# NumericalEarth/Breeze.jl

Measured on AMD Instinct MI355X. Metric: grid-cells advanced/sec (tendency+Poisson step), 512^3 anelastic, higher is better.
Workload: dtype f64

## Files before the change

breeze.jl_amd/csrc/bz_tendency5_kernels.h:

```cpp
#pragma once
#include "bz_internal.h"
#include "bz_weno.h"
#include "bz_tendency3_kernels.h"

#ifndef BZ_KO
#define BZ_KO 0
#endif
#ifndef BZ6_ROTATE_DUTY
#define BZ6_ROTATE_DUTY 0
#endif
#ifndef BZ6_UNROLL2
#define BZ6_UNROLL2 0
#endif
#ifndef BZ6_LDS_BARRIER
#define BZ6_LDS_BARRIER 0
#endif
__device__ __forceinline__ void bz6_barrier()
{
#if BZ6_LDS_BARRIER
    __builtin_amdgcn_fence(__ATOMIC_RELEASE, "workgroup", "local");
    __builtin_amdgcn_s_barrier();
    __builtin_amdgcn_fence(__ATOMIC_ACQUIRE, "workgroup", "local");
#else
    __syncthreads();
#endif
}
typedef long long ix_t;
typedef unsigned ix32_t;

struct LevRow5 {
    double rho, rrho;
    double rho_f, rrho_f;
    double Ax, Ay, Vinv_c;
    double pi;
    double Vinv_f, T_r;
    double pad[6];
};
struct Lev5 {
    const LevRow5 *p;
#ifdef __HIPCC__
    __device__ __forceinline__ double at(int k, int f) const { return ((ColPtr::cptr)(const double *)p)[(long long)k * 16 + f]; }
    __device__ __forceinline__ double rho(int k) const { return at(k, 0); }
    __device__ __forceinline__ double rrho(int k) const { return at(k, 1); }
    __device__ __forceinline__ double rho_f(int k) const { return at(k, 2); }
    __device__ __forceinline__ double rrho_f(int k) const { return at(k, 3); }
    __device__ __forceinline__ double Ax(int k) const { return at(k, 4); }
    __device__ __forceinline__ double Ay(int k) const { return at(k, 5); }
    __device__ __forceinline__ double Vinv_c(int k) const { return at(k, 6); }
    __device__ __forceinline__ double pi(int k) const { return at(k, 7); }
    __device__ __forceinline__ double Vinv_f(int k) const { return at(k, 8); }
// ... 197 lines not shown
    {
        const double rh = g.rho[kbeg], rr = g.rrho[kbeg];
        bool z0 = (b[3] == 0.0);
#pragma unroll
        for (int q = 0; q < HPT; ++q)
            if (hok[q]) {
                T[0][0][hr[q]][hc[q]] = bz_cdiv(pa[hn[q]], rh, rr);
                if constexpr (Q) {
                    const double hbv = bz_cdiv(pb[hn[q]], rh, rr);
                    T[0][1][hr[q]][hc[q]] = hbv;
                    z0 = z0 && (hbv == 0.0);
                }
            }
        if (ZS && !__all(z0) && tx == 0) ZF[0] = 0;
    }
    __syncthreads();

    double ea = 0.0, eb = 0.0;
    int buf = 0;
    double ru_n = ru[n], rv_n = rv[n], rw_n = rw[n + sz];
    double rvtop_n = (tyu == 0 || (Q && tyu == TY / 2)) ? rv[ntop0] : 0.0;
    double ta_nx = 0.0, tb_nx = 0.0;
    if constexpr (BZ5_TOPS_AHEAD) { ta_nx = pa[n + 3 * sz]; if constexpr (Q) tb_nx = pb[n + 3 * sz]; }
    for (int k = kbeg; k < kend; ++k, n += sz) {
        double ha[HPT], hb[HPT];
        const unsigned lev = (unsigned)(k + 1 - kbeg) * sz;
        double ta_raw, tb_raw = 0.0;
        if constexpr (BZ5_TOPS_AHEAD) {
            ta_raw = ta_nx; tb_raw = tb_nx;
            const unsigned up = (k + 4 <= g.Nz + g.Hz - 1) ? 4 * sz : 3 * sz;
            ta_nx = pa[n + up];
            if constexpr (Q) tb_nx = pb[n + up];
        } else { ta_raw = pa[n + 3 * sz]; if constexpr (Q) tb_raw = pb[n + 3 * sz]; }
        const int lv3 = (ZS || (Q && BZ5_RAW_LDS)) ? (k - kbeg) % 3 : 0;
        bool zxy = false;
        if constexpr (ZS) {
            if (t == 0) ZF[(lv3 + 2) % 3] = 1;
            zxy = __builtin_amdgcn_readfirstlane(ZF[lv3]) != 0;
        }
#pragma unroll
        for (int q = 0; q < HPT; ++q) {
            if (BZ_KO & 2) { ha[q] = ta_raw; hb[q] = tb_raw; }
            else { ha[q] = hok[q] ? pa[hn[q] + lev] : 0.0; hb[q] = (Q && hok[q]) ? pb[hn[q] + lev] : 0.0; }
        }
        const double u0a = (BZ_KO & 16) ? ta_raw : (E.mode == 2) ? E.u0[n] : 0.0, u0b = (BZ_KO & 16) ? tb_raw : (Q && E.mode == 2) ? E.u0b[n] : 0.0;
        const double ru_t = ru_n, rv_t = rv_n, rw_t = rw_n, rvtop = rvtop_n;
        const int turn = (k - kbeg) & (TY - 1);
        const bool duty_a = tyu == turn, duty_b = Q && tyu == ((turn + TY / 2) & (TY - 1));
        if (BZ_KO & 32) { ru_n = ta_raw * 1e-3; rv_n = tb_raw; rw_n = ta_raw * 1e-4; } else {
        ru_n = ru[n + sz]; rv_n = rv[n + sz]; rw_n = rw[n + 2 * sz]; }
        {
            const int turn_n = (turn + 1) & (TY - 1);
            const bool duty_n = tyu == turn_n || (Q && tyu == ((turn_n + TY / 2) & (TY - 1)));
            rvtop_n = duty_n ? rv[ntop0 + lev] : 0.0;
        }
        const double rho = LV.rho(k), rrho = LV.rrho(k), Ax_k = LV.Ax(k), Ay_k = LV.Ay(k), Vi_k = LV.Vinv_c(k);
        const double rho1 = LV.rho(k + 1), rrho1 = LV.rrho(k + 1), rhof1 = LV.rho_f(k + 1), rrhof1 = LV.rrho_f(k + 1);
        const double rho3 = LV.rho(k + 3), rrho3 = LV.rrho(k + 3);
        if (((k - kbeg) & (BZ5_EB - 1)) == 0) {
            const int kk = min(k + (tx & (BZ5_EB - 1)), kend - 1);
            const long long ne = g.idx(ie, jc, kk);
            const double rhk = g.rho[kk], rrk = g.rrho[kk];
            const double ue = bz_cdiv(ru[ne], rhk, rrk);
            const bool le_ = ue > 0.0;
            const double cf = g.Ax[kk] * ue;
            ea = rhk * (cf * bz_up5(bz_cdiv(pa[ne - 3], rhk, rrk), bz_cdiv(pa[ne - 2], rhk, rrk), bz_cdiv(pa[ne - 1], rhk, rrk),
                                    bz_cdiv(pa[ne], rhk, rrk), bz_cdiv(pa[ne + 1], rhk, rrk), bz_cdiv(pa[ne + 2], rhk, rrk), le_));
            if constexpr (Q)
            eb = rhk * (cf * bz_up5(bz_cdiv(pb[ne - 3], rhk, rrk), bz_cdiv(pb[ne - 2], rhk, rrk), bz_cdiv(pb[ne - 1], rhk, rrk),
                                    bz_cdiv(pb[ne], rhk, rrk), bz_cdiv(pb[ne + 1], rhk, rrk), bz_cdiv(pb[ne + 2], rhk, rrk), le_));
        }
        const int src = (k - kbeg) & (BZ5_EB - 1);
        const double ut = bz_cdiv(ru_t, rho, rrho), vt = bz_cdiv(rv_t, rho, rrho);
        const double wt = bz_cdiv(rw_t, rhof1, rrhof1);
        const double cfx = Ax_k * ut, cfy = Ay_k * vt, cfz = g.Az * wt, rf = rhof1;
        const bool lx = ut > 0.0, ly = vt > 0.0, lz = wt > 0.0;
        const int Bz = bz_buffer_face(k + 1, g.Nz);
        double cfy2 = 0.0;
        bool ly2 = false;
        if (duty_a || duty_b) {
            const double vtop = bz_cdiv(rvtop, rho, rrho);
            ly2 = vtop > 0.0;
            cfy2 = Ay_k * vtop;
        }
        const int c = tx + 3;
        double fxa, fya, fza_hi, fxb, fyb, fzb_hi;
        const double ta = bz_cdiv(ta_raw, rho3, rrho3);
        {
            const double(*Tk)[TC] = T[buf][0];
            const double *rr_ = Tk[ty + 3] + tx;
            fxa = rho * (cfx * bz_up5(rr_[0], rr_[1], rr_[2], a[3], rr_[4], rr_[5], lx));
            fya = rho * (cfy * bz_up5y<WY>(Tk[ty][c], Tk[ty + 1][c], Tk[ty + 2][c], a[3], Tk[ty + 4][c], Tk[ty + 5][c], ly, Byj));
            FY[buf][0][ty][tx] = fya;
            if (duty_a)
                FY[buf][0][TY][tx] = rho * (cfy2 * bz_up5y<WY>(Tk[TY][c], Tk[TY + 1][c], Tk[TY + 2][c], Tk[TY + 3][c], Tk[TY + 4][c], Tk[TY + 5][c], ly2, Byt));
            fza_hi = rf * (cfz * bz_upB(a[1], a[2], a[3], a[4], a[5], ta, lz, Bz));
        }
        double tb = 0.0;
        fxb = 0.0; fyb = 0.0; fzb_hi = 0.0;
        if constexpr (Q) {
// ... 55 lines not shown
            const double ga = -(Vi * ((na - fxa) + dya + (fza_hi - fza)));
            double gb = 0.0;
            if constexpr (Q) {
                double nb = __shfl_down(fxb, 1);
                const double xb = __shfl(eb, src);
                if (tx == le) nb = xb;
                const double dyb = FY[buf][1][ty + 1][tx] - fyb;
                gb = -(Vi * ((nb - fxb) + dyb + (fzb_hi - fzb)));
            }
            if (store) {
                const double rth = bz_rk_apply_pre(E.mode, E.dt, E.alpha, E.oma, u0a, E.u0_out, ga, pa_n, n);
                F.oa[n] = rth;
                if constexpr (Q) {
                    const double rq = bz_rk_apply_pre(E.mode, E.dt, E.alpha, E.oma, u0b, E.u0b_out, gb, pb_n, n);
                    F.ob[n] = rq;
                }
            }
        }
        fza = fza_hi; fzb = fzb_hi;
#pragma unroll
        for (int s = 0; s < 5; ++s) { a[s] = a[s + 1]; b[s] = b[s + 1]; }
        a[5] = ta; b[5] = tb;
        buf ^= 1;
    }
}


template <bool DRYQ, bool GUARD>
__device__ __forceinline__ bool bz_lean_skip(const Lean5 &F)
{
    if constexpr (!GUARD) return false;
    const bool dry = F.qstate != nullptr && __builtin_amdgcn_readfirstlane(*F.qstate) == 1;
    return dry != DRYQ;
}
template <int TY, bool WY = false, bool DRYQ = false, bool GUARD = true>
__global__ __launch_bounds__(64 * TY) __attribute__((amdgpu_waves_per_eu(BZ5_SCALAR_WAVES, BZ5_SCALAR_WAVES))) void k5_scalar_pair(DevGrid g, Lean5 F, int kchunk, RKEpilogue E)
{
    constexpr int TR = TY + 6, TC = 72;
    __shared__ double T[2 * 2 * TR * TC];
    __shared__ double FY[2 * 2 * (TY + 1) * 64];
    __shared__ int ZF[3];
    __shared__ double RAW[(!DRYQ && BZ5_RAW_LDS) ? 3 * 2 * 64 * TY : 1];
    if (bz_lean_skip<DRYQ, GUARD>(F)) return;
    k5_scalar_pair_body<TY, WY, DRYQ>(g, F, kchunk, E, T, FY, ZF, RAW);
}

template <int KIND>
__device__ __forceinline__ double flux_x_lean(const DevGrid &g, const Tend3Fields &F, const double *__restrict__ m, int i, int j, int k, int By = 3)
{
    const long long n = g.idx(i, j, k);
    const double a = (KIND == T3_V && By != 3) ? bz_symm2(g.Ax[k] * F.ru[n - g.Sx], g.Ax[k] * F.ru[n]) : adv_x<KIND>(g, F, n, k);
    const double rh = (KIND == T3_W) ? g.rho_f[k] : g.rho[k], rr = (KIND == T3_W) ? g.rrho_f[k] : g.rrho[k];
    if constexpr (KIND == T3_U)
        return a * bz_up5(bz_cdiv(m[n - 2], rh, rr), bz_cdiv(m[n - 1], rh, rr), bz_cdiv(m[n], rh, rr), bz_cdiv(m[n + 1], rh, rr),
                          bz_cdiv(m[n + 2], rh, rr), bz_cdiv(m[n + 3], rh, rr), a > 0.0);
    else
        return a * bz_up5(bz_cdiv(m[n - 3], rh, rr), bz_cdiv(m[n - 2], rh, rr), bz_cdiv(m[n - 1], rh, rr), bz_cdiv(m[n], rh, rr),
                          bz_cdiv(m[n + 1], rh, rr), bz_cdiv(m[n + 2], rh, rr), a > 0.0);
}


template <int TY, bool MF = false, bool WY = false, bool ST = false>
__global__ __launch_bounds__(64 * TY, BZ_LEAN_WAVES) void k6_u(DevGrid g, Lean5 L, int kchunk, RKEpilogue E)
{
    static_assert(!(ST && WY), "stored-velocity instantiations: periodic / slab rows");
    constexpr int TR = TY + 6, TC = 72, NT = 64 * TY;
    constexpr int NH1 = TR * 70 - TY * 64;
    constexpr int NH2 = 3 * (TY + 1) + 64 + 3 * TY;
    static_assert(NH1 <= NT && NH2 <= NT, "one frame cell of each kind per thread");
    __shared__ double U[2][TR][TC];
    __shared__ double RU[2][TY][TC];
    __shared__ double RV[2][TY + 1][TC];
    __shared__ double RW[2][TY][TC];
    __shared__ double FY[2][TY + 1][64];
    int bx, by, bz;
    bz_block5(L, bx, by, bz);
    const int tx = threadIdx.x, ty = threadIdx.y, t = ty * 64 + tx, tc = tx + 3;
    const int i0 = bx * 64, j0 = by * TY;
    const int i = i0 + tx, j = j0 + ty;
    const int ic = min(i, g.Nx + 2), jc = min(j, g.Ny + 2);
    const int ie = i0 - 1, le = 0;
    const int kbeg = bz * kchunk, kend = min(kbeg + kchunk, g.Nz);
    if (kbeg >= kend) return;
    const ix_t sz = (ix_t)g.Sxy;
    const bool store = (i < g.Nx) && (j < g.Ny);
    const double *__restrict__ ru = L.ru, *__restrict__ rv = L.rv, *__restrict__ rw = L.rw;
    const double *__restrict__ vel = ST ? L.vel : L.ru;
    Tend3Fields F;
    F.ru = L.ru; F.rv = L.rv; F.rw = L.rw; F.u = F.v = F.w = F.T = F.q = nullptr; F.c = ST ? L.vel : nullptr; F.G = L.out;
    ix_t n = (ix_t)g.idx(ic, jc, kbeg);
    const bool h1ok = !(BZ_KO & 32768) && t < NH1;
    int h1r = 0, h1c = 0;
    {
        const int h = h1ok ? t : 0;
        if (h < 6 * 70) { const int rr = h / 70; h1c = h - rr * 70; h1r = (rr < 3) ? rr : TY + rr; }
        else { const int hh = h - 6 * 70, rr = hh / 6, cc = hh - rr * 6; h1r = 3 + rr; h1c = (cc < 3) ? cc : 64 + cc; }
    }
    const ix_t h1n = (ix_t)g.idx(min(i0 - 3 + h1c, g.Nx + 2), min(j0 - 3 + h1r, g.Ny + 2), kbeg);
    const bool h1raw = h1ok && h1r >= 3 && h1r < TY + 3 && (h1c == 2 || h1c == 67 || h1c == 68);
    const bool h2ok = !(BZ_KO & 32768) && t < NH2;
    int h2sel = 0, h2r = 0, h2c = 0;
    {
        const int id = h2ok ? t : 0;
        if (id < 3 * (TY + 1)) { h2r = id / 3; const int cc = id - 3 * h2r; h2c = (cc < 2) ? 1 + cc : 67; }
        else if (id < 3 * (TY + 1) + 64) { h2r = TY; h2c = 3 + (id - 3 * (TY + 1)); }
        else { h2sel = 1; const int m = id - 3 * (TY + 1) - 64; h2r = m / 3; const int cc = m - 3 * h2r; h2c = (cc < 2) ? 1 + cc : 67; }
    }
    const double *__restrict__ h2src = h2sel ? rw : rv;
    const ix_t h2n = (ix_t)g.idx(min(i0 - 3 + h2c, g.Nx + 2), min(j0 + h2r, g.Ny + 2), kbeg) + (h2sel ? sz : (ix_t)0);

    double r[6];
#pragma unroll
    for (int s = 0; s < 6; ++s) r[s] = ST ? vel[n + s * sz - 3 * sz] : bz_cdiv(ru[n + s * sz - 3 * sz], g.rho[kbeg + s - 3], g.rrho[kbeg + s - 3]);
    double fz_lo = vflux<T3_U>(g, F, n, kbeg, r[0], r[1], r[2], r[3], r[4], r[5]);
    double q0 = ru[n], q1 = ru[n + sz], q2 = ru[n + 2 * sz];
    U[0][ty + 3][tc] = r[3];
    RU[0][ty][tc] = q0;
    RV[0][ty][tc] = rv[n];
    RW[0][ty][tc] = rw[n + sz];
    if (h1ok) {
        const double raw = (ST && !h1raw) ? 0.0 : ru[h1n];
        U[0][h1r][h1c] = ST ? vel[h1n] : bz_cdiv(raw, g.rho[kbeg], g.rrho[kbeg]);
        if (h1raw) RU[0][h1r - 3][h1c] = raw;
    }
    if (h2ok) { if (h2sel) RW[0][h2r][h2c] = h2src[h2n]; else RV[0][h2r][h2c] = h2src[h2n]; }
    double tcur_raw = ru[n + 3 * sz];
    double tcur_v = ST ? vel[n + 3 * sz] : 0.0;
    double u0cur = (E.mode == 2) ? E.u0[n] : 0.0;
    __syncthreads();

    double edge = 0.0;
    int buf = 0;
#if BZ6_UNROLL2
#pragma unroll 2
#endif
    for (int k = kbeg; k < kend; ++k, n += sz) {
        const ix_t lev1 = (ix_t)(k + 1 - kbeg) * sz;
        const double p_top = ST ? ru[n + sz] : ru[n + ((k + 4 <= g.Nz + g.Hz - 1) ? 4 * sz : 3 * sz)];
        const double p_topv = ST ? vel[n + ((k + 4 <= g.Nz + g.Hz - 1) ? 4 * sz : 3 * sz)] : 0.0;
        const double p_h1 = (BZ_KO & 256) ? p_top : h1ok ? (ST ? vel : ru)[h1n + lev1] : 0.0;
        const double p_h1raw = (ST && h1raw) ? ru[h1n + lev1] : 0.0;
        const double p_h2 = (BZ_KO & 512) ? p_top : h2ok ? h2src[h2n + lev1] : 0.0;
        const double p_rv = (BZ_KO & 1024) ? p_top * 0.5 : rv[n + sz], p_rw = (BZ_KO & 1024) ? p_top * 0.25 : rw[n + 2 * sz];
        const double p_u0 = (BZ_KO & 2048) ? p_top : (E.mode == 2) ? E.u0[n + sz] : 0.0;
        if (((k - kbeg) & (BZ5_EB - 1)) == 0) {
            const int kk = min(k + (tx & (BZ5_EB - 1)), kend - 1);
            edge = ST ? flux_x_at<T3_U>(g, F, ie, jc, kk) : flux_x_lean<T3_U>(g, F, ru, ie, jc, kk);
        }
        const int src = (k - kbeg) & (BZ5_EB - 1);
        const double Ax = g.Ax[k], Ay = g.Ay[k], Az = g.Az;
        const double c0 = r[3];
        const double(*Uk)[TC] = U[buf];
        const double *rur = RU[buf][ty] + tc, *ur = Uk[ty + 3] + tc;
        const double ax = bz_symm4(Ax * rur[-1], Ax * q0, Ax * rur[1], Ax * rur[2]);
        const double fx = ax * bz_up5(ur[-2], ur[-1], c0, ur[1], ur[2], ur[3], ax > 0.0);
        const double *rvr = RV[buf][ty] + tc;
        const double ay = bz_symm4(Ay * rvr[-2], Ay * rvr[-1], Ay * rvr[0], Ay * rvr[1]);
        const double fy = ay * bz_up5y<WY>(Uk[ty][tc], Uk[ty + 1][tc], Uk[ty + 2][tc], c0, Uk[ty + 4][tc], Uk[ty + 5][tc], ay > 0.0, by5_face<WY>(g, __builtin_amdgcn_readfirstlane(j)));
        FY[buf][ty][tx] = fy;
        if (ty == (BZ6_ROTATE_DUTY ? ((k - kbeg) & (TY - 1)) : 0) && !(BZ_KO & 4096)) {
            const double *rvt = RV[buf][TY] + tc;
            const double at = bz_symm4(Ay * rvt[-2], Ay * rvt[-1], Ay * rvt[0], Ay * rvt[1]);
            FY[buf][TY][tx] = at * bz_up5y<WY>(Uk[TY][tc], Uk[TY + 1][tc], Uk[TY + 2][tc], Uk[TY + 3][tc], Uk[TY + 4][tc], Uk[TY + 5][tc], at > 0.0,
                                               by5_face<WY>(g, j0 + TY));
        }
        const double tnew = ST ? tcur_v : bz_cdiv(tcur_raw, g.rho[k + 3], g.rrho[k + 3]);
        const double *rwr = RW[buf][ty] + tc;
        const double wt = bz_symm4(Az * rwr[-2], Az * rwr[-1], Az * rwr[0], Az * rwr[1]);
        const double fz_hi = wt * bz_upB(r[1], r[2], r[3], r[4], r[5], tnew, wt > 0.0, bz_buffer_face(k + 1, g.Nz));
        U[buf ^ 1][ty + 3][tc] = r[4];
        RU[buf ^ 1][ty][tc] = ST ? p_top : q1;
        RV[buf ^ 1][ty][tc] = p_rv;
        RW[buf ^ 1][ty][tc] = p_rw;
        if (h1ok) {
            U[buf ^ 1][h1r][h1c] = ST ? p_h1 : bz_cdiv(p_h1, g.rho[k + 1], g.rrho[k + 1]);
            if (h1raw) RU[buf ^ 1][h1r - 3][h1c] = ST ? p_h1raw : p_h1;
        }
        if (h2ok) { if (h2sel) RW[buf ^ 1][h2r][h2c] = p_h2; else RV[buf ^ 1][h2r][h2c] = p_h2; }
        if (!(BZ_KO & 16384) && (!(BZ_KO & 8192) || ((k - kbeg) & 1))) bz6_barrier();
        {
            double nb = __shfl_up(fx, 1);
            const double e = __shfl(edge, src);
            if (tx == le) nb = e;
            const double dx = fx - nb;
            const double dy = (BZ_KO & 16384) ? 0.5 * fy : FY[buf][ty + 1][tx] - fy;
            double Gu = -(g.Vinv_c[k] * (dx + dy + (fz_hi - fz_lo)));
            if constexpr (MF) {
                if (L.mforce & 1) {
                    const double *rv0 = RV[buf][ty] + tc, *rv1 = RV[buf][ty + 1] + tc;
                    const double a = (rv0[-1] + rv1[-1]) / 2, b = (rv0[0] + rv1[0]) / 2;
                    Gu -= -L.cor_f * ((a + b) / 2);
                }
                if (L.mforce & (2 | 8)) {
                    const double rho = g.rho[k];
                    double tot = (L.mforce & 8) ? rho * L.Su[k] : 0.0;
                    if (L.mforce & 2) tot = (L.mforce & 8) ? tot + rho * L.Fu[k] : rho * L.Fu[k];
                    Gu += tot;
                }
            }
            if (store) L.out[n] = (ST && E.mode == 0) ? Gu : bz_rk_apply_pre(E.mode, E.dt, E.alpha, E.oma, u0cur, E.u0_out, Gu, q0, n);
        }
        fz_lo = fz_hi;
#pragma unroll
        for (int s = 0; s < 5; ++s) r[s] = r[s + 1];
        r[5] = tnew;
        if (ST) q0 = p_top;
        else { q0 = q1; q1 = q2; q2 = tcur_raw; tcur_raw = p_top; }
        u0cur = p_u0;
        if (ST) tcur_v = p_topv;
        buf ^= 1;
    }
}


template <int TY, bool MF = false, bool WY = false, bool ST = false>
__global__ __launch_bounds__(64 * TY, ((MF && WY) ? 4 : BZ_LEAN_WAVES)) void k6_v(DevGrid g, Lean5 L, int kchunk, RKEpilogue E)
{
    static_assert(!(ST && WY), "stored-velocity instantiations: periodic / slab rows");
    constexpr int RV = TY + 6, RM = TY + 4;
    constexpr int TC = 72;
    __shared__ double Tv[2][RV][TC];
    __shared__ double Tm[2][3][RM][64];
    __shared__ double FY[2][TY + 1][64];
    constexpr int NT = 64 * TY, NFR = 16 * 64, HPT = (NFR + NT - 1) / NT;
    int bx, by, bz;
    bz_block5(L, bx, by, bz);
    const int tx = threadIdx.x, ty = threadIdx.y, t = ty * 64 + tx, tc = tx + 3;
    const int i0 = bx * 64, j0 = by * TY;
    const int i = i0 + tx, j = j0 + ty;
    const int ic = min(i, g.Nx + 2), jc = min(j, g.Ny + 2);
    const int nact = min(64, g.Nx - i0);
    const int ie = i0 + nact, le = nact - 1;
    const int kbeg = bz * kchunk, kend = min(kbeg + kchunk, g.Nz);
    if (kbeg >= kend) return;
    const ix_t sz = (ix_t)g.Sxy;
    const bool store = (i < g.Nx) && (j < g.Ny) && !(WY && j == 0);
    const int ju = __builtin_amdgcn_readfirstlane(j);
    const int Bf = by5_face<WY>(g, ju), Bc = by5_center<WY>(g, ju), Bc0 = by5_center<WY>(g, j0 - 1);
    const double *__restrict__ ru = L.ru, *__restrict__ rv = L.rv, *__restrict__ rw = L.rw;
    const double *__restrict__ vel = ST ? L.vel : L.rv;
    Tend3Fields F;
    F.ru = L.ru; F.rv = L.rv; F.rw = L.rw; F.u = F.v = F.w = F.T = F.q = nullptr; F.c = ST ? L.vel : nullptr; F.G = L.out;
    const double Az = g.Az;
    ix_t n = (ix_t)g.idx(ic, jc, kbeg);

    bool hok[HPT];
    int hsel[HPT], hrow[HPT];
    ix_t hn[HPT];
    const double *hsrc[HPT];
#pragma unroll
    for (int q = 0; q < HPT; ++q) {
        const int h = t + q * NT;
        hok[q] = h < NFR;
        const int id = __builtin_amdgcn_readfirstlane(hok[q] ? (h >> 6) : 0);
        int sel, row, grow;
        if (id < 6) { sel = 0; row = (id < 3) ? id : TY + id; grow = j0 - 3 + row; }
        else if (id < 9) { sel = 1; const int m = id - 6; row = (m < 2) ? m : TY + 2; grow = j0 - 2 + row; }
        else if (id < 13) { sel = 2; const int m = id - 9; row = (m < 2) ? m : TY + m; grow = j0 - 2 + row; }
        else { sel = 3; const int m = id - 13; row = (m < 2) ? m : TY + 2; grow = j0 - 2 + row; }
        hsel[q] = sel; hrow[q] = row;
        hsrc[q] = (sel == 1) ? ru : (sel == 3) ? rw : (ST && sel == 0) ? vel : rv;
        hn[q] = (ix_t)g.idx(min(i0 + tx, g.Nx + 2), min(grow, g.Ny + 2), kbeg) + (sel == 3 ? sz : (ix_t)0);
    }
    auto frame_load = [&](int q, ix_t lev) -> double { return hsrc[q][hn[q] + lev]; };
    auto frame_store = [&](int b, int q, double raw, int klev) {
        if (hsel[q] == 0) Tv[b][hrow[q]][tc] = ST ? raw : bz_cdiv(raw, g.rho[klev], g.rrho[klev]);
        else Tm[b][hsel[q] - 1][hrow[q]][tx] = ((hsel[q] == 1) ? g.Ax[klev] : (hsel[q] == 2) ? g.Ay[klev] : Az) * raw;
    };

    const bool sok = t < 5 * TY;
    const int srow = sok ? t / 5 : 0, scc = sok ? t % 5 : 0, scol = (scc < 3) ? scc : 64 + scc;
    const ix_t sn = (ix_t)g.idx(min(i0 - 3 + scol, g.Nx + 2), min(j0 + srow, g.Ny + 2), kbeg);

    double r[6];
#pragma unroll
    for (int s = 0; s < 6; ++s) r[s] = ST ? vel[n + s * sz - 3 * sz] : bz_cdiv(rv[n + s * sz - 3 * sz], g.rho[kbeg + s - 3], g.rrho[kbeg + s - 3]);
    double fz_lo;
    if (WY && Bf != 3) {
        const double wt0 = bz_symm2(Az * rw[n - (ix_t)g.Sx], Az * rw[n]);
        fz_lo = wt0 * bz_upB(r[0], r[1], r[2], r[3], r[4], r[5], wt0 > 0.0, bz_buffer_face(kbeg, g.Nz));
    } else fz_lo = vflux<T3_V>(g, F, n, kbeg, r[0], r[1], r[2], r[3], r[4], r[5]);
    double q0 = rv[n], q1 = rv[n + sz], q2 = rv[n + 2 * sz];
    Tv[0][ty + 3][tc] = r[3];
    if (sok) Tv[0][srow + 3][scol] = ST ? vel[sn] : bz_cdiv(rv[sn], g.rho[kbeg], g.rrho[kbeg]);
    Tm[0][0][ty + 2][tx] = g.Ax[kbeg] * ru[n];
    Tm[0][1][ty + 2][tx] = g.Ay[kbeg] * q0;
    Tm[0][2][ty + 2][tx] = Az * rw[n + sz];
#pragma unroll
    for (int q = 0; q < HPT; ++q)
        if (hok[q]) frame_store(0, q, frame_load(q, 0), kbeg);
    __syncthreads();

    double tcur_raw = rv[n + 3 * sz];
    double tcur_v = ST ? vel[n + 3 * sz] : 0.0;
    double u0cur = (E.mode == 2) ? E.u0[n] : 0.0;
    double edge = 0.0;
    int buf = 0;
    for (int k = kbeg; k < kend; ++k, n += sz) {
        const ix_t lev = (ix_t)(k + 1 - kbeg) * sz;
        double hnext[HPT];
#pragma unroll
        for (int q = 0; q < HPT; ++q) hnext[q] = hok[q] ? frame_load(q, lev) : 0.0;
        const double p_side = sok ? (ST ? vel : rv)[sn + lev] : 0.0;
        const double p_top = ST ? rv[n + sz] : rv[n + ((k + 4 <= g.Nz + g.Hz - 1) ? 4 * sz : 3 * sz)];
        const double p_topv = ST ? vel[n + ((k + 4 <= g.Nz + g.Hz - 1) ? 4 * sz : 3 * sz)] : 0.0;
        const double p_u0 = (E.mode == 2) ? E.u0[n + sz] : 0.0;
        const double tnew_raw = tcur_raw, u0v = u0cur;
        const double ru_n = g.Ax[k + 1] * ru[n + sz], rw_n = Az * rw[n + 2 * sz];
        double cor_u = 0.0, cg1 = 0.0, cg3 = 0.0;
        if constexpr (MF) { if ((L.mforce & 1) && tx == 63) { const ix_t sy = (ix_t)g.Sx; cg1 = ru[n - sy + 1]; cg3 = ru[n + 1]; } }
        if (((k - kbeg) & (BZ5_EB - 1)) == 0) {
            const int kk = min(k + (tx & (BZ5_EB - 1)), kend - 1);
            edge = ST ? flux_x_at<T3_V>(g, F, ie, jc, kk) : flux_x_lean<T3_V>(g, F, rv, ie, jc, kk, Bf);
        }
        const int src = (k - kbeg) & (BZ5_EB - 1);
        const double rho = g.rho[k];
        const double c0 = r[3];
        const double(*V)[TC] = Tv[buf];
        const double *vrow = V[ty + 3] + tc;
        const double(*MU)[64] = Tm[buf][0];
        const double(*MV)[64] = Tm[buf][1];
        const double(*MW)[64] = Tm[buf][2];
        const double ut = bz_symm4y<WY>(MU[ty][tx], MU[ty + 1][tx], MU[ty + 2][tx], MU[ty + 3][tx], Bf);
        const double fx = ut * bz_up5(vrow[-3], vrow[-2], vrow[-1], c0, vrow[1], vrow[2], ut > 0.0);
        const double vt = (!WY || Bc == 3) ? bz_symm4(MV[ty + 1][tx], MV[ty + 2][tx], MV[ty + 3][tx], MV[ty + 4][tx]) : bz_symm2(MV[ty + 2][tx], MV[ty + 3][tx]);
        const double fy = vt * bz_up5y<WY>(V[ty + 1][tc], V[ty + 2][tc], c0, V[ty + 4][tc], V[ty + 5][tc], V[ty + 6][tc], vt > 0.0, Bc);
        FY[buf][ty + 1][tx] = fy;
        if (ty == 0 && !(BZ_KO & 4096)) {
            const double vb = (!WY || Bc0 == 3) ? bz_symm4(MV[0][tx], MV[1][tx], MV[2][tx], MV[3][tx]) : bz_symm2(MV[1][tx], MV[2][tx]);
            FY[buf][0][tx] = vb * bz_up5y<WY>(V[0][tc], V[1][tc], V[2][tc], V[3][tc], V[4][tc], V[5][tc], vb > 0.0, Bc0);
        }
        const double tnew = ST ? tcur_v : bz_cdiv(tnew_raw, g.rho[k + 3], g.rrho[k + 3]);
        const double wt = bz_symm4y<WY>(MW[ty][tx], MW[ty + 1][tx], MW[ty + 2][tx], MW[ty + 3][tx], Bf);
        const double fz_hi = wt * bz_upB(r[1], r[2], r[3], r[4], r[5], tnew, wt > 0.0, bz_buffer_face(k + 1, g.Nz));
        if constexpr (MF) {
            if (L.mforce & 1) {
                const double Axk = g.Ax[k];
                const double l1 = MU[ty + 1][tx + 1], l3 = MU[ty + 2][tx + 1];
                const double c1 = (tx == 63) ? Axk * cg1 : l1, c3 = (tx == 63) ? Axk * cg3 : l3;
                cor_u = (((MU[ty + 1][tx] + c1) / 2 + (MU[ty + 2][tx] + c3) / 2) / 2) / Axk;
            }
        }
        Tv[buf ^ 1][ty + 3][tc] = r[4];
        if (sok) Tv[buf ^ 1][srow + 3][scol] = ST ? p_side : bz_cdiv(p_side, g.rho[k + 1], g.rrho[k + 1]);
        Tm[buf ^ 1][0][ty + 2][tx] = ru_n;
        Tm[buf ^ 1][1][ty + 2][tx] = g.Ay[k + 1] * (ST ? p_top : q1);
        Tm[buf ^ 1][2][ty + 2][tx] = rw_n;
#pragma unroll
        for (int q = 0; q < HPT; ++q)
            if (hok[q]) frame_store(buf ^ 1, q, hnext[q], k + 1);
        bz6_barrier();
        {
            double nb = __shfl_down(fx, 1);
            const double e = __shfl(edge, src);
            if (tx == le) nb = e;
            const double dx = nb - fx;
            const double dy = fy - FY[buf][ty][tx];
            double Gv = -(g.Vinv_c[k] * (dx + dy + (fz_hi - fz_lo)));
            if constexpr (MF) {
                if (L.mforce & 1) Gv -= L.cor_f * cor_u;
                if (L.mforce & (4 | 16)) {
                    double tot = (L.mforce & 16) ? rho * L.Sv[k] : 0.0;
                    if (L.mforce & 4) tot = (L.mforce & 16) ? tot + rho * L.Fv[k] : rho * L.Fv[k];
                    Gv += tot;
                }
            }
            if (store) L.out[n] = (ST && E.mode == 0) ? Gv : bz_rk_apply_pre(E.mode, E.dt, E.alpha, E.oma, u0v, E.u0_out, Gv, q0, n);
            if constexpr (WY) {
                if (i < g.Nx && j == 0) L.out[n] = 0.0;
                if (i < g.Nx && j == g.Ny - 1) L.out[n + (ix_t)g.Sx] = 0.0;
            }
        }
        fz_lo = fz_hi;
        if (ST) q0 = p_top;
        else { q0 = q1; q1 = q2; q2 = tnew_raw; tcur_raw = p_top; }
        u0cur = p_u0;
        if (ST) tcur_v = p_topv;
#pragma unroll
        for (int s = 0; s < 5; ++s) r[s] = r[s + 1];
        r[5] = tnew;
        buf ^= 1;
    }
}

__device__ __forceinline__ double buoyancy5(const DevGrid &g, double rth, double rq, int k, double rho, double rrho, double pi, double T_ref)
{
    const double th = bz_cdiv(rth, rho, rrho), q = bz_cdiv(rq, rho, rrho);
    double T;
    if (__all(q == 0.0)) T = pi * th;
    else {
        const double qd = 1.0 - q;
        const double cpm = qd * g.cpd + q * g.cpv;
        T = bz_exner_factor(g, k, q, cpm) * th;
    }
    const double Rm = (1.0 - q) * g.Rd + q * g.Rv;
    const double rhop = rho * (g.Rd * T_ref / (Rm * T) - 1.0);
    return -g.g * rhop;
}


template <int TY, bool WY = false, bool DRYQ = false, bool GUARD = true, int BM = 4>
__global__ __launch_bounds__(64 * TY, BZ6_W_WAVES) void k6_w(DevGrid g, Lean5 L, int kchunk, RKEpilogue E)
{
    constexpr bool ST = BM != 4;
    static_assert(!(ST && (WY || DRYQ || GUARD)), "stored-velocity instantiations: periodic / slab rows, no moisture-scan dispatch");
// ... 54 lines not shown
        qv[s] = Ayk * rv[n + s * sz - 2 * sz];
        qt[s] = top ? Ayk * rv[ntop0 + s * sz - 2 * sz] : 0.0;
    }
    double fz_lo, b_lo, r_lo = 0.0;
    {
        const int B = bz_buffer_center(kbeg - 1, g.Nz);
        const double wt = (B == 3) ? bz_symm4(qw[0], qw[1], qw[2], qw[3]) : bz_symm2(qw[1], qw[2]);
        fz_lo = wt * bz_upB(wr[0], wr[1], wr[2], wr[3], wr[4], wr[5], wt > 0.0, B);
        if constexpr (BM == 4) b_lo = buoyancy5(g, pa[n - sz], dryq ? 0.0 : pb[n - sz], kbeg - 1, LV.rho(kbeg - 1), LV.rrho(kbeg - 1), LV.pi(kbeg - 1), LV.T_r(kbeg - 1));
        else if constexpr (BM == 0) b_lo = buoyancy3(g, bT[n - sz], bq[n - sz], kbeg - 1);
        else if constexpr (BM == 3) b_lo = bz_buoyancy(g, bT, bq, (long long)(n - sz), kbeg - 1);
        else if constexpr (BM == 2) { b_lo = bT[n - sz] - g.p_r[kbeg - 1]; r_lo = bq[n - sz] - g.rho[kbeg - 1]; }
        else b_lo = 0.0;
    }
    T[0][ty + 3][tc] = wr[3];
    if (hok) T[0][hr][hc] = ST ? vel[hn] : bz_cdiv(rw[hn], LV.rho_f(kbeg), LV.rrho_f(kbeg));
    double tcur_raw = rw[n + 3 * sz];
    double tcur_v = ST ? vel[n + 3 * sz] : 0.0;
    double u0cur = (E.mode == 2) ? E.u0[n] : 0.0;
    __syncthreads();

    double edge = 0.0;
    int buf = 0;
    for (int k = kbeg; k < kend; ++k, n += sz) {
        const ix32_t lev = (ix32_t)(k - kbeg) * sz;
        const double p_h = hok ? (ST ? vel : rw)[hn + lev + sz] : 0.0;
        const double p_top = rw[n + ((k + 4 <= g.Nz + g.Hz) ? 4 * sz : 3 * sz)];
        const double p_topv = ST ? vel[n + ((k + 4 <= g.Nz + g.Hz) ? 4 * sz : 3 * sz)] : 0.0;
        const double Tcur = (BM == 1) ? 0.0 : (ST ? bT : pa)[n], rqcur = (BM == 1) ? 0.0 : ST ? bq[n] : dryq ? 0.0 : pb[n];
        const double p_u0 = (E.mode == 2) ? E.u0[n + sz] : 0.0;
        const double Axn = ST ? g.Ax[k + 2] : LV.Ax(k + 2), Ayn = ST ? g.Ay[k + 2] : LV.Ay(k + 2);
        const double qun = Axn * ru[n + 2 * sz], qvn = Ayn * rv[n + 2 * sz];
        const double qtn = top ? Ayn * rv[ntop0 + lev + 2 * sz] : 0.0;
        if (((k - kbeg) & (BZ5_EB - 1)) == 0) {
            const int kk = min(k + (tx & (BZ5_EB - 1)), kend - 1);
            edge = ST ? flux_x_at<T3_W>(g, F, ie, jc, kk) : flux_x_lean<T3_W>(g, F, rw, ie, jc, kk);
        }
        const int src = (k - kbeg) & (BZ5_EB - 1);
        const int Bf = bz_buffer_face(k, g.Nz);
        const double w0 = wr[3];
        const double qwnew = Az * (ST ? rw[n + 2 * sz] : raw2);
        const double uold = ST ? rw[n] : raw0;
        const double(*Tk)[TC] = T[buf];
        const double *wrow = Tk[ty + 3] + tc;
        const double ut = (Bf == 3) ? bz_symm4(qu[0], qu[1], qu[2], qu[3]) : bz_symm2(qu[1], qu[2]);
        const double fx = ut * bz_up5(wrow[-3], wrow[-2], wrow[-1], w0, wrow[1], wrow[2], ut > 0.0);
        const double vt = (Bf == 3) ? bz_symm4(qv[0], qv[1], qv[2], qv[3]) : bz_symm2(qv[1], qv[2]);
        const double fy = vt * bz_up5y<WY>(Tk[ty][tc], Tk[ty + 1][tc], Tk[ty + 2][tc], w0, Tk[ty + 4][tc], Tk[ty + 5][tc], vt > 0.0, by5_face<WY>(g, __builtin_amdgcn_readfirstlane(j)));
        FY[buf][ty][tx] = fy;
        if (top && !(BZ_KO & 4096)) {
            const double v2 = (Bf == 3) ? bz_symm4(qt[0], qt[1], qt[2], qt[3]) : bz_symm2(qt[1], qt[2]);
            FY[buf][TY][tx] = v2 * bz_up5y<WY>(Tk[TY][tc], Tk[TY + 1][tc], Tk[TY + 2][tc], Tk[TY + 3][tc], Tk[TY + 4][tc], Tk[TY + 5][tc], v2 > 0.0,
                                               by5_face<WY>(g, j0 + TY));
        }
        const double wnew = ST ? tcur_v : bz_cdiv(tcur_raw, LV.rho_f(k + 3), LV.rrho_f(k + 3));
        double fz_hi;
        {
            const int B = bz_buffer_center(k, g.Nz);
            const double wt = (B == 3) ? bz_symm4(qw[1], qw[2], qw[3], qwnew) : bz_symm2(qw[2], qw[3]);
            fz_hi = wt * bz_upB(wr[1], wr[2], wr[3], wr[4], wr[5], wnew, wt > 0.0, B);
        }
        double b_hi = 0.0, r_hi = 0.0;
        if constexpr (BM == 4) b_hi = buoyancy5(g, Tcur, rqcur, k, LV.rho(k), LV.rrho(k), LV.pi(k), LV.T_r(k));
        else if constexpr (BM == 0) b_hi = buoyancy3(g, Tcur, rqcur, k);
        else if constexpr (BM == 3) b_hi = bz_buoyancy(g, bT, bq, (long long)n, k);
        else if constexpr (BM == 2) { b_hi = Tcur - g.p_r[k]; r_hi = rqcur - g.rho[k]; }
        T[buf ^ 1][ty + 3][tc] = wr[4];
        if (hok) T[buf ^ 1][hr][hc] = ST ? p_h : bz_cdiv(p_h, LV.rho_f(k + 1), LV.rrho_f(k + 1));
        bz6_barrier();
        {
            double nb = __shfl_down(fx, 1);
            const double e = __shfl(edge, src);
            if (tx == le) nb = e;
            const double dx = nb - fx;
            const double dy = FY[buf][ty + 1][tx] - fy;
            const double adv = -((ST ? g.Vinv_f[k] : LV.Vinv_f(k)) * (dx + dy + (fz_hi - fz_lo)));
            double Gval;
            if constexpr (BM == 2) Gval = adv - (b_hi - b_lo) * g.rdzf[k] - g.g * ((r_hi + r_lo) / 2.0);
            else if constexpr (BM == 1) Gval = adv;
            else Gval = adv + 0.5 * (b_lo + b_hi);
            if (store)
                L.out[n] = (ST && E.mode == 0) ? Gval : bz_rk_apply_pre(E.mode, E.dt, E.alpha, E.oma, u0cur, E.u0_out, Gval, uold, n);
        }
        fz_lo = fz_hi;
        b_lo = b_hi;
        r_lo = r_hi;
#pragma unroll
        for (int s = 0; s < 3; ++s) { qu[s] = qu[s + 1]; qv[s] = qv[s + 1]; qt[s] = qt[s + 1]; qw[s] = qw[s + 1]; }
        qu[3] = qun; qv[3] = qvn; qt[3] = qtn; qw[3] = qwnew;
        raw0 = raw1; raw1 = raw2; raw2 = tcur_raw;
        tcur_raw = p_top; u0cur = p_u0;
        if (ST) tcur_v = p_topv;
#pragma unroll
        for (int s = 0; s < 5; ++s) wr[s] = wr[s + 1];
        wr[5] = wnew;
        buf ^= 1;
    }
}
```

Baseline: 4.231 billion.

## Split vertical march into interior specialization and prescale LDS momentum tiles

After: 4.268 billion (median of 6 runs). About the same (+0.9%).

```diff
diff --git a/breeze.jl_amd/csrc/bz_tendency5_kernels.h b/breeze.jl_amd/csrc/bz_tendency5_kernels.h
--- a/breeze.jl_amd/csrc/bz_tendency5_kernels.h
+++ b/breeze.jl_amd/csrc/bz_tendency5_kernels.h
@@ -14,6 +14,11 @@
 #endif
 #ifndef BZ6_LDS_BARRIER
 #define BZ6_LDS_BARRIER 0
+#endif
+#if BZ6_UNROLL2
+#define BZ6_UNROLL_PRAGMA _Pragma("unroll 2")
+#else
+#define BZ6_UNROLL_PRAGMA
 #endif
 __device__ __forceinline__ void bz6_barrier()
 {
@@ -26,6 +31,22 @@
 #endif
 }
 typedef long long ix_t;
+#ifndef BZ_INTERIOR_SPLIT
+#define BZ_INTERIOR_SPLIT (sizeof(double) == 8)
+#endif
+template <bool V> struct bz_flag { static constexpr bool value = V; };
+#define BZ_LEVEL_LAMBDA(I, k) [&](auto I, const int k) __attribute__((always_inline))
+#define BZ_MARCH(SPLIT, level, k, kbeg, kend, lo, hi, STEP)                                           \
+    for (int k = (kbeg); k < (kend);) {                                                               \
+        if constexpr (BZ_INTERIOR_SPLIT && (SPLIT)) if (k >= (lo)) {                                                      \
+            const int ke_ = min((kend), (hi) + 1);                                                    \
+            BZ6_UNROLL_PRAGMA                                                                         \
+            for (; k < ke_; ++k, STEP) level(bz_flag<true>{}, k);                                     \
+            if (k >= (kend)) break;                                                                   \
+        }                                                                                             \
+        level(bz_flag<false>{}, k);                                                                   \
+        ++k, STEP;                                                                                    \
+    }
 typedef unsigned ix32_t;
 
 struct LevRow5 {
@@ -269,13 +290,14 @@
     double rvtop_n = (tyu == 0 || (Q && tyu == TY / 2)) ? rv[ntop0] : 0.0;
     double ta_nx = 0.0, tb_nx = 0.0;
     if constexpr (BZ5_TOPS_AHEAD) { ta_nx = pa[n + 3 * sz]; if constexpr (Q) tb_nx = pb[n + 3 * sz]; }
-    for (int k = kbeg; k < kend; ++k, n += sz) {
+    auto level = BZ_LEVEL_LAMBDA(I, k) {
+        constexpr bool INTERIOR = decltype(I)::value;
         double ha[HPT], hb[HPT];
         const unsigned lev = (unsigned)(k + 1 - kbeg) * sz;
         double ta_raw, tb_raw = 0.0;
         if constexpr (BZ5_TOPS_AHEAD) {
             ta_raw = ta_nx; tb_raw = tb_nx;
-            const unsigned up = (k + 4 <= g.Nz + g.Hz - 1) ? 4 * sz : 3 * sz;
+            const unsigned up = (INTERIOR || k + 4 <= g.Nz + g.Hz - 1) ? 4 * sz : 3 * sz;
             ta_nx = pa[n + up];
             if constexpr (Q) tb_nx = pb[n + up];
         } else { ta_raw = pa[n + 3 * sz]; if constexpr (Q) tb_raw = pb[n + 3 * sz]; }
@@ -322,7 +344,7 @@
         const double wt = bz_cdiv(rw_t, rhof1, rrhof1);
         const double cfx = Ax_k * ut, cfy = Ay_k * vt, cfz = g.Az * wt, rf = rhof1;
         const bool lx = ut > 0.0, ly = vt > 0.0, lz = wt > 0.0;
-        const int Bz = bz_buffer_face(k + 1, g.Nz);
+        const int Bz = INTERIOR ? 3 : bz_buffer_face(k + 1, g.Nz);
         double cfy2 = 0.0;
         bool ly2 = false;
         if (duty_a || duty_b) {
@@ -424,7 +446,8 @@
         for (int s = 0; s < 5; ++s) { a[s] = a[s + 1]; b[s] = b[s + 1]; }
         a[5] = ta; b[5] = tb;
         buf ^= 1;
-    }
+    };
+    BZ_MARCH(true, level, k, kbeg, kend, 2, g.Nz - 4, n += sz)
 }
 
 
@@ -470,6 +493,7 @@
     constexpr int NH1 = TR * 70 - TY * 64;
     constexpr int NH2 = 3 * (TY + 1) + 64 + 3 * TY;
     static_assert(NH1 <= NT && NH2 <= NT, "one frame cell of each kind per thread");
+    constexpr bool PS = !MF && !ST;
     __shared__ double U[2][TR][TC];
     __shared__ double RU[2][TY][TC];
     __shared__ double RV[2][TY + 1][TC];
@@ -488,6 +512,7 @@
     const bool store = (i < g.Nx) && (j < g.Ny);
     const double *__restrict__ ru = L.ru, *__restrict__ rv = L.rv, *__restrict__ rw = L.rw;
     const double *__restrict__ vel = ST ? L.vel : L.ru;
+    const Lev5 LV{L.lev};
     Tend3Fields F;
     F.ru = L.ru; F.rv = L.rv; F.rw = L.rw; F.u = F.v = F.w = F.T = F.q = nullptr; F.c = ST ? L.vel : nullptr; F.G = L.out;
     ix_t n = (ix_t)g.idx(ic, jc, kbeg);
@@ -516,16 +541,22 @@
     for (int s = 0; s < 6; ++s) r[s] = ST ? vel[n + s * sz - 3 * sz] : bz_cdiv(ru[n + s * sz - 3 * sz], g.rho[kbeg + s - 3], g.rrho[kbeg + s - 3]);
     double fz_lo = vflux<T3_U>(g, F, n, kbeg, r[0], r[1], r[2], r[3], r[4], r[5]);
     double q0 = ru[n], q1 = ru[n + sz], q2 = ru[n + 2 * sz];
-    U[0][ty + 3][tc] = r[3];
-    RU[0][ty][tc] = q0;
-    RV[0][ty][tc] = rv[n];
-    RW[0][ty][tc] = rw[n + sz];
-    if (h1ok) {
-        const double raw = (ST && !h1raw) ? 0.0 : ru[h1n];
-        U[0][h1r][h1c] = ST ? vel[h1n] : bz_cdiv(raw, g.rho[kbeg], g.rrho[kbeg]);
-        if (h1raw) RU[0][h1r - 3][h1c] = raw;
-    }
-    if (h2ok) { if (h2sel) RW[0][h2r][h2c] = h2src[h2n]; else RV[0][h2r][h2c] = h2src[h2n]; }
+    {
+        const double Ax0 = ST ? g.Ax[kbeg] : LV.Ax(kbeg), Ay0 = ST ? g.Ay[kbeg] : LV.Ay(kbeg), Az0 = g.Az;
+        U[0][ty + 3][tc] = r[3];
+        RU[0][ty][tc] = PS ? Ax0 * q0 : q0;
+        RV[0][ty][tc] = PS ? Ay0 * rv[n] : rv[n];
+        RW[0][ty][tc] = PS ? Az0 * rw[n + sz] : rw[n + sz];
+        if (h1ok) {
+            const double raw = (ST && !h1raw) ? 0.0 : ru[h1n];
+            U[0][h1r][h1c] = ST ? vel[h1n] : bz_cdiv(raw, g.rho[kbeg], g.rrho[kbeg]);
+            if (h1raw) RU[0][h1r - 3][h1c] = PS ? Ax0 * raw : raw;
+        }
+        if (h2ok) {
+            const double x = h2src[h2n];
+            if (h2sel) RW[0][h2r][h2c] = PS ? Az0 * x : x; else RV[0][h2r][h2c] = PS ? Ay0 * x : x;
+        }
+    }
     double tcur_raw = ru[n + 3 * sz];
     double tcur_v = ST ? vel[n + 3 * sz] : 0.0;
     double u0cur = (E.mode == 2) ? E.u0[n] : 0.0;
@@ -533,13 +564,12 @@
 
     double edge = 0.0;
     int buf = 0;
-#if BZ6_UNROLL2
-#pragma unroll 2
-#endif
-    for (int k = kbeg; k < kend; ++k, n += sz) {
+    auto level = BZ_LEVEL_LAMBDA(I, k) {
+        constexpr bool INTERIOR = decltype(I)::value;
         const ix_t lev1 = (ix_t)(k + 1 - kbeg) * sz;
-        const double p_top = ST ? ru[n + sz] : ru[n + ((k + 4 <= g.Nz + g.Hz - 1) ? 4 * sz : 3 * sz)];
-        const double p_topv = ST ? vel[n + ((k + 4 <= g.Nz + g.Hz - 1) ? 4 * sz : 3 * sz)] : 0.0;
+        const ix_t up = (INTERIOR || k + 4 <= g.Nz + g.Hz - 1) ? 4 * sz : 3 * sz;
+        const double p_top = ST ? ru[n + sz] : ru[n + up];
+        const double p_topv = ST ? vel[n + up] : 0.0;
         const double p_h1 = (BZ_KO & 256) ? p_top : h1ok ? (ST ? vel : ru)[h1n + lev1] : 0.0;
         const double p_h1raw = (ST && h1raw) ? ru[h1n + lev1] : 0.0;
         const double p_h2 = (BZ_KO & 512) ? p_top : h2ok ? h2src[h2n + lev1] : 0.0;
@@ -550,35 +580,37 @@
             edge = ST ? flux_x_at<T3_U>(g, F, ie, jc, kk) : flux_x_lean<T3_U>(g, F, ru, ie, jc, kk);
         }
         const int src = (k - kbeg) & (BZ5_EB - 1);
-        const double Ax = g.Ax[k], Ay = g.Ay[k], Az = g.Az;
+        const double Ax = ST ? g.Ax[k] : LV.Ax(k), Ay = ST ? g.Ay[k] : LV.Ay(k), Az = g.Az, Vi = ST ? g.Vinv_c[k] : LV.Vinv_c(k);
+        const double rho1 = ST ? 0.0 : LV.rho(k + 1), rrho1 = ST ? 0.0 : LV.rrho(k + 1), rho3 = ST ? 0.0 : LV.rho(k + 3), rrho3 = ST ? 0.0 : LV.rrho(k + 3);
+        const double Ax1 = !PS ? 0.0 : ST ? g.Ax[k + 1] : LV.Ax(k + 1), Ay1 = !PS ? 0.0 : ST ? g.Ay[k + 1] : LV.Ay(k + 1);
         const double c0 = r[3];
         const double(*Uk)[TC] = U[buf];
         const double *rur = RU[buf][ty] + tc, *ur = Uk[ty + 3] + tc;
-        const double ax = bz_symm4(Ax * rur[-1], Ax * q0, Ax * rur[1], Ax * rur[2]);
+        const double ax = PS ? bz_symm4(rur[-1], Ax * q0, rur[1], rur[2]) : bz_symm4(Ax * rur[-1], Ax * q0, Ax * rur[1], Ax * rur[2]);
         const double fx = ax * bz_up5(ur[-2], ur[-1], c0, ur[1], ur[2], ur[3], ax > 0.0);
         const double *rvr = RV[buf][ty] + tc;
-        const double ay = bz_symm4(Ay * rvr[-2], Ay * rvr[-1], Ay * rvr[0], Ay * rvr[1]);
+        const double ay = PS ? bz_symm4(rvr[-2], rvr[-1], rvr[0], rvr[1]) : bz_symm4(Ay * rvr[-2], Ay * rvr[-1], Ay * rvr[0], Ay * rvr[1]);
         const double fy = ay * bz_up5y<WY>(Uk[ty][tc], Uk[ty + 1][tc], Uk[ty + 2][tc], c0, Uk[ty + 4][tc], Uk[ty + 5][tc], ay > 0.0, by5_face<WY>(g, __builtin_amdgcn_readfirstlane(j)));
         FY[buf][ty][tx] = fy;
         if (ty == (BZ6_ROTATE_DUTY ? ((k - kbeg) & (TY - 1)) : 0) && !(BZ_KO & 4096)) {
             const double *rvt = RV[buf][TY] + tc;
-            const double at = bz_symm4(Ay * rvt[-2], Ay * rvt[-1], Ay * rvt[0], Ay * rvt[1]);
+            const double at = PS ? bz_symm4(rvt[-2], rvt[-1], rvt[0], rvt[1]) : bz_symm4(Ay * rvt[-2], Ay * rvt[-1], Ay * rvt[0], Ay * rvt[1]);
             FY[buf][TY][tx] = at * bz_up5y<WY>(Uk[TY][tc], Uk[TY + 1][tc], Uk[TY + 2][tc], Uk[TY + 3][tc], Uk[TY + 4][tc], Uk[TY + 5][tc], at > 0.0,
                                                by5_face<WY>(g, j0 + TY));
         }
-        const double tnew = ST ? tcur_v : bz_cdiv(tcur_raw, g.rho[k + 3], g.rrho[k + 3]);
+        const double tnew = ST ? tcur_v : bz_cdiv(tcur_raw, rho3, rrho3);
         const double *rwr = RW[buf][ty] + tc;
-        const double wt = bz_symm4(Az * rwr[-2], Az * rwr[-1], Az * rwr[0], Az * rwr[1]);
-        const double fz_hi = wt * bz_upB(r[1], r[2], r[3], r[4], r[5], tnew, wt > 0.0, bz_buffer_face(k + 1, g.Nz));
+        const double wt = PS ? bz_symm4(rwr[-2], rwr[-1], rwr[0], rwr[1]) : bz_symm4(Az * rwr[-2], Az * rwr[-1], Az * rwr[0], Az * rwr[1]);
+        const double fz_hi = wt * bz_upB(r[1], r[2], r[3], r[4], r[5], tnew, wt > 0.0, INTERIOR ? 3 : bz_buffer_face(k + 1, g.Nz));
         U[buf ^ 1][ty + 3][tc] = r[4];
-        RU[buf ^ 1][ty][tc] = ST ? p_top : q1;
-        RV[buf ^ 1][ty][tc] = p_rv;
-        RW[buf ^ 1][ty][tc] = p_rw;
+        RU[buf ^ 1][ty][tc] = PS ? Ax1 * (ST ? p_top : q1) : (ST ? p_top : q1);
+        RV[buf ^ 1][ty][tc] = PS ? Ay1 * p_rv : p_rv;
+        RW[buf ^ 1][ty][tc] = PS ? Az * p_rw : p_rw;
         if (h1ok) {
-            U[buf ^ 1][h1r][h1c] = ST ? p_h1 : bz_cdiv(p_h1, g.rho[k + 1], g.rrho[k + 1]);
-            if (h1raw) RU[buf ^ 1][h1r - 3][h1c] = ST ? p_h1raw : p_h1;
-        }
-        if (h2ok) { if (h2sel) RW[buf ^ 1][h2r][h2c] = p_h2; else RV[buf ^ 1][h2r][h2c] = p_h2; }
+            U[buf ^ 1][h1r][h1c] = ST ? p_h1 : bz_cdiv(p_h1, rho1, rrho1);
+            if (h1raw) RU[buf ^ 1][h1r - 3][h1c] = PS ? Ax1 * (ST ? p_h1raw : p_h1) : (ST ? p_h1raw : p_h1);
+        }
+        if (h2ok) { if (h2sel) RW[buf ^ 1][h2r][h2c] = PS ? Az * p_h2 : p_h2; else RV[buf ^ 1][h2r][h2c] = PS ? Ay1 * p_h2 : p_h2; }
         if (!(BZ_KO & 16384) && (!(BZ_KO & 8192) || ((k - kbeg) & 1))) bz6_barrier();
         {
             double nb = __shfl_up(fx, 1);
@@ -586,7 +618,7 @@
             if (tx == le) nb = e;
             const double dx = fx - nb;
             const double dy = (BZ_KO & 16384) ? 0.5 * fy : FY[buf][ty + 1][tx] - fy;
-            double Gu = -(g.Vinv_c[k] * (dx + dy + (fz_hi - fz_lo)));
+            double Gu = -(Vi * (dx + dy + (fz_hi - fz_lo)));
             if constexpr (MF) {
                 if (L.mforce & 1) {
                     const double *rv0 = RV[buf][ty] + tc, *rv1 = RV[buf][ty + 1] + tc;
@@ -594,7 +626,7 @@
                     Gu -= -L.cor_f * ((a + b) / 2);
                 }
                 if (L.mforce & (2 | 8)) {
-                    const double rho = g.rho[k];
+                    const double rho = ST ? g.rho[k] : LV.rho(k);
                     double tot = (L.mforce & 8) ? rho * L.Su[k] : 0.0;
                     if (L.mforce & 2) tot = (L.mforce & 8) ? tot + rho * L.Fu[k] : rho * L.Fu[k];
                     Gu += tot;
@@ -611,7 +643,8 @@
         u0cur = p_u0;
         if (ST) tcur_v = p_topv;
         buf ^= 1;
-    }
+    };
+    BZ_MARCH(!ST, level, k, kbeg, kend, 2, g.Nz - 4, n += sz)
 }
 
 
@@ -641,6 +674,8 @@
     const int Bf = by5_face<WY>(g, ju), Bc = by5_center<WY>(g, ju), Bc0 = by5_center<WY>(g, j0 - 1);
     const double *__restrict__ ru = L.ru, *__restrict__ rv = L.rv, *__restrict__ rw = L.rw;
     const double *__restrict__ vel = ST ? L.vel : L.rv;
+    const Lev5 LV{L.lev};
+    constexpr bool LT = ST || (MF && WY);
     Tend3Fields F;
     F.ru = L.ru; F.rv = L.rv; F.rw = L.rw; F.u = F.v = F.w = F.T = F.q = nullptr; F.c = ST ? L.vel : nullptr; F.G = L.out;
     const double Az = g.Az;
@@ -665,9 +700,9 @@
         hn[q] = (ix_t)g.idx(min(i0 + tx, g.Nx + 2), min(grow, g.Ny + 2), kbeg) + (sel == 3 ? sz : (ix_t)0);
     }
     auto frame_load = [&](int q, ix_t lev) -> double { return hsrc[q][hn[q] + lev]; };
-    auto frame_store = [&](int b, int q, double raw, int klev) {
-        if (hsel[q] == 0) Tv[b][hrow[q]][tc] = ST ? raw : bz_cdiv(raw, g.rho[klev], g.rrho[klev]);
-        else Tm[b][hsel[q] - 1][hrow[q]][tx] = ((hsel[q] == 1) ? g.Ax[klev] : (hsel[q] == 2) ? g.Ay[klev] : Az) * raw;
+    auto frame_store = [&](int b, int q, double raw, double rho_l, double rrho_l, double Ax_l, double Ay_l) {
+        if (hsel[q] == 0) Tv[b][hrow[q]][tc] = ST ? raw : bz_cdiv(raw, rho_l, rrho_l);
+        else Tm[b][hsel[q] - 1][hrow[q]][tx] = ((hsel[q] == 1) ? Ax_l : (hsel[q] == 2) ? Ay_l : Az) * raw;
     };
 
     const bool sok = t < 5 * TY;
@@ -690,7 +725,7 @@
     Tm[0][2][ty + 2][tx] = Az * rw[n + sz];
 #pragma unroll
     for (int q = 0; q < HPT; ++q)
-        if (hok[q]) frame_store(0, q, frame_load(q, 0), kbeg);
+        if (hok[q]) frame_store(0, q, frame_load(q, 0), g.rho[kbeg], g.rrho[kbeg], g.Ax[kbeg], g.Ay[kbeg]);
     __syncthreads();
 
     double tcur_raw = rv[n + 3 * sz];
@@ -698,17 +733,23 @@
     double u0cur = (E.mode == 2) ? E.u0[n] : 0.0;
     double edge = 0.0;
     int buf = 0;
-    for (int k = kbeg; k < kend; ++k, n += sz) {
+    auto level = BZ_LEVEL_LAMBDA(I, k) {
+        constexpr bool INTERIOR = decltype(I)::value;
         const ix_t lev = (ix_t)(k + 1 - kbeg) * sz;
         double hnext[HPT];
 #pragma unroll
         for (int q = 0; q < HPT; ++q) hnext[q] = hok[q] ? frame_load(q, lev) : 0.0;
         const double p_side = sok ? (ST ? vel : rv)[sn + lev] : 0.0;
-        const double p_top = ST ? rv[n + sz] : rv[n + ((k + 4 <= g.Nz + g.Hz - 1) ? 4 * sz : 3 * sz)];
-        const double p_topv = ST ? vel[n + ((k + 4 <= g.Nz + g.Hz - 1) ? 4 * sz : 3 * sz)] : 0.0;
+        const ix_t up = (INTERIOR || k + 4 <= g.Nz + g.Hz - 1) ? 4 * sz : 3 * sz;
+        const double p_top = ST ? rv[n + sz] : rv[n + up];
+        const double p_topv = ST ? vel[n + up] : 0.0;
         const double p_u0 = (E.mode == 2) ? E.u0[n + sz] : 0.0;
         const double tnew_raw = tcur_raw, u0v = u0cur;
-        const double ru_n = g.Ax[k + 1] * ru[n + sz], rw_n = Az * rw[n + 2 * sz];
+        const double Vi = LT ? g.Vinv_c[k] : LV.Vinv_c(k);
+        const double rho1 = ST ? 0.0 : LT ? g.rho[k + 1] : LV.rho(k + 1), rrho1 = ST ? 0.0 : LT ? g.rrho[k + 1] : LV.rrho(k + 1);
+        const double rho3 = ST ? 0.0 : LT ? g.rho[k + 3] : LV.rho(k + 3), rrho3 = ST ? 0.0 : LT ? g.rrho[k + 3] : LV.rrho(k + 3);
+        const double Ax1 = LT ? g.Ax[k + 1] : LV.Ax(k + 1), Ay1 = LT ? g.Ay[k + 1] : LV.Ay(k + 1);
+        const double ru_n = Ax1 * ru[n + sz], rw_n = Az * rw[n + 2 * sz];
         double cor_u = 0.0, cg1 = 0.0, cg3 = 0.0;
         if constexpr (MF) { if ((L.mforce & 1) && tx == 63) { const ix_t sy = (ix_t)g.Sx; cg1 = ru[n - sy + 1]; cg3 = ru[n + 1]; } }
         if (((k - kbeg) & (BZ5_EB - 1)) == 0) {
@@ -716,7 +757,7 @@
             edge = ST ? flux_x_at<T3_V>(g, F, ie, jc, kk) : flux_x_lean<T3_V>(g, F, rv, ie, jc, kk, Bf);
         }
         const int src = (k - kbeg) & (BZ5_EB - 1);
-        const double rho = g.rho[k];
+        const double rho = !MF ? 0.0 : LT ? g.rho[k] : LV.rho(k);
         const double c0 = r[3];
         const double(*V)[TC] = Tv[buf];
         const double *vrow = V[ty + 3] + tc;
@@ -732,25 +773,25 @@
             const double vb = (!WY || Bc0 == 3) ? bz_symm4(MV[0][tx], MV[1][tx], MV[2][tx], MV[3][tx]) : bz_symm2(MV[1][tx], MV[2][tx]);
             FY[buf][0][tx] = vb * bz_up5y<WY>(V[0][tc], V[1][tc], V[2][tc], V[3][tc], V[4][tc], V[5][tc], vb > 0.0, Bc0);
         }
-        const double tnew = ST ? tcur_v : bz_cdiv(tnew_raw, g.rho[k + 3], g.rrho[k + 3]);
+        const double tnew = ST ? tcur_v : bz_cdiv(tnew_raw, rho3, rrho3);
         const double wt = bz_symm4y<WY>(MW[ty][tx], MW[ty + 1][tx], MW[ty + 2][tx], MW[ty + 3][tx], Bf);
-        const double fz_hi = wt * bz_upB(r[1], r[2], r[3], r[4], r[5], tnew, wt > 0.0, bz_buffer_face(k + 1, g.Nz));
+        const double fz_hi = wt * bz_upB(r[1], r[2], r[3], r[4], r[5], tnew, wt > 0.0, INTERIOR ? 3 : bz_buffer_face(k + 1, g.Nz));
         if constexpr (MF) {
             if (L.mforce & 1) {
-                const double Axk = g.Ax[k];
+                const double Axk = LT ? g.Ax[k] : LV.Ax(k);
                 const double l1 = MU[ty + 1][tx + 1], l3 = MU[ty + 2][tx + 1];
                 const double c1 = (tx == 63) ? Axk * cg1 : l1, c3 = (tx == 63) ? Axk * cg3 : l3;
                 cor_u = (((MU[ty + 1][tx] + c1) / 2 + (MU[ty + 2][tx] + c3) / 2) / 2) / Axk;
             }
         }
         Tv[buf ^ 1][ty + 3][tc] = r[4];
-        if (sok) Tv[buf ^ 1][srow + 3][scol] = ST ? p_side : bz_cdiv(p_side, g.rho[k + 1], g.rrho[k + 1]);
+        if (sok) Tv[buf ^ 1][srow + 3][scol] = ST ? p_side : bz_cdiv(p_side, rho1, rrho1);
         Tm[buf ^ 1][0][ty + 2][tx] = ru_n;
-        Tm[buf ^ 1][1][ty + 2][tx] = g.Ay[k + 1] * (ST ? p_top : q1);
+        Tm[buf ^ 1][1][ty + 2][tx] = Ay1 * (ST ? p_top : q1);
         Tm[buf ^ 1][2][ty + 2][tx] = rw_n;
 #pragma unroll
         for (int q = 0; q < HPT; ++q)
-            if (hok[q]) frame_store(buf ^ 1, q, hnext[q], k + 1);
+            if (hok[q]) frame_store(buf ^ 1, q, hnext[q], rho1, rrho1, Ax1, Ay1);
         bz6_barrier();
         {
             double nb = __shfl_down(fx, 1);
@@ -758,7 +799,7 @@
             if (tx == le) nb = e;
             const double dx = nb - fx;
             const double dy = fy - FY[buf][ty][tx];
-            double Gv = -(g.Vinv_c[k] * (dx + dy + (fz_hi - fz_lo)));
+            double Gv = -(Vi * (dx + dy + (fz_hi - fz_lo)));
             if constexpr (MF) {
                 if (L.mforce & 1) Gv -= L.cor_f * cor_u;
                 if (L.mforce & (4 | 16)) {
@@ -782,7 +823,8 @@
         for (int s = 0; s < 5; ++s) r[s] = r[s + 1];
         r[5] = tnew;
         buf ^= 1;
-    }
+    };
+    BZ_MARCH((TY == 16 && !MF), level, k, kbeg, kend, 2, g.Nz - 4, n += sz)
 }
 
 __device__ __forceinline__ double buoyancy5(const DevGrid &g, double rth, double rq, int k, double rho, double rrho, double pi, double T_ref)
@@ -883,11 +925,13 @@
 
     double edge = 0.0;
     int buf = 0;
-    for (int k = kbeg; k < kend; ++k, n += sz) {
+    auto level = BZ_LEVEL_LAMBDA(I, k) {
+        constexpr bool INTERIOR = decltype(I)::value;
         const ix32_t lev = (ix32_t)(k - kbeg) * sz;
         const double p_h = hok ? (ST ? vel : rw)[hn + lev + sz] : 0.0;
-        const double p_top = rw[n + ((k + 4 <= g.Nz + g.Hz) ? 4 * sz : 3 * sz)];
-        const double p_topv = ST ? vel[n + ((k + 4 <= g.Nz + g.Hz) ? 4 * sz : 3 * sz)] : 0.0;
+        const ix32_t up = (INTERIOR || k + 4 <= g.Nz + g.Hz) ? 4 * sz : 3 * sz;
+        const double p_top = rw[n + up];
+        const double p_topv = ST ? vel[n + up] : 0.0;
         const double Tcur = (BM == 1) ? 0.0 : (ST ? bT : pa)[n], rqcur = (BM == 1) ? 0.0 : ST ? bq[n] : dryq ? 0.0 : pb[n];
         const double p_u0 = (E.mode == 2) ? E.u0[n + sz] : 0.0;
         const double Axn = ST ? g.Ax[k + 2] : LV.Ax(k + 2), Ayn = ST ? g.Ay[k + 2] : LV.Ay(k + 2);
@@ -898,7 +942,7 @@
             edge = ST ? flux_x_at<T3_W>(g, F, ie, jc, kk) : flux_x_lean<T3_W>(g, F, rw, ie, jc, kk);
         }
         const int src = (k - kbeg) & (BZ5_EB - 1);
-        const int Bf = bz_buffer_face(k, g.Nz);
+        const int Bf = INTERIOR ? 3 : bz_buffer_face(k, g.Nz);
         const double w0 = wr[3];
         const double qwnew = Az * (ST ? rw[n + 2 * sz] : raw2);
         const double uold = ST ? rw[n] : raw0;
@@ -917,7 +961,7 @@
         const double wnew = ST ? tcur_v : bz_cdiv(tcur_raw, LV.rho_f(k + 3), LV.rrho_f(k + 3));
         double fz_hi;
         {
-            const int B = bz_buffer_center(k, g.Nz);
+            const int B = INTERIOR ? 3 : bz_buffer_center(k, g.Nz);
             const double wt = (B == 3) ? bz_symm4(qw[1], qw[2], qw[3], qwnew) : bz_symm2(qw[2], qw[3]);
             fz_hi = wt * bz_upB(wr[1], wr[2], wr[3], wr[4], wr[5], wnew, wt > 0.0, B);
         }
@@ -956,5 +1000,6 @@
         for (int s = 0; s < 5; ++s) wr[s] = wr[s + 1];
         wr[5] = wnew;
         buf ^= 1;
-    }
-}
+    };
+    BZ_MARCH((BM == 4), level, k, kbeg, kend, 3, g.Nz - 3, n += sz)
+}
```
